# Fool-Yang/AlphaSnake-Zero

Hardware: AMD Instinct MI355X
Metric: self-play env-steps/sec (11x11, 4 snakes, 50 MCTS sims) (higher is better)
Workload: dtype f32 (tower convolutions: each f32 operand split into f16 hi + lo, 3 f16 MFMAs per product, f32 accumulate)

## Files before the change

### alphasnake-zero_amd/csrc/conv_split.hip

```cpp
#include "common.h"
#include "train_fold.h"
#include <stdlib.h>

typedef float f32x16 __attribute__((ext_vector_type(16)));
typedef _Float16 f16x8 __attribute__((ext_vector_type(8)));
typedef _Float16 f16x4 __attribute__((ext_vector_type(4)));
typedef __bf16 bf16x8 __attribute__((ext_vector_type(8)));
typedef unsigned uint4_t __attribute__((ext_vector_type(4)));
typedef int i32x4 __attribute__((ext_vector_type(4)));
typedef int i32x8 __attribute__((ext_vector_type(8)));
typedef short s16x2 __attribute__((ext_vector_type(2)));

template <bool BF> __device__ __forceinline__ float hs_from16(_Float16 v)
{
    if (BF) return (float)__builtin_bit_cast(__bf16, v);
    return (float)v;
}
template <bool BF> __device__ __forceinline__ _Float16 hs_to16(float v)
{
    if (BF) return __builtin_bit_cast(_Float16, (__bf16)v);
    return (_Float16)__builtin_amdgcn_fmed3f(v, -65504.f, 65504.f);
}

#define HS_C 128
// ... 1407 lines not shown
    SNK_REQUIRE(n_layers >= 1 && n_layers <= HS_RECT_MAX_LAYERS, "snk_conv_rect_plan: %d layers (at most %d)", n_layers, HS_RECT_MAX_LAYERS);
    const long mb = rect_max_blocks(n_images, height, width, act16);
    SNK_REQUIRE(mb >= 0 && mb < (1l << 31), "snk_conv_rect_plan: bad shape %d x %d x %d", n_images, height, width);
    if (n_images == 0) return 0;
    RectPlanArgs a;
    a.n_layers = n_layers;
    for (int i = 0; i < n_layers; ++i) {
        SNK_REQUIRE(grow[i] >= 0 && grow[i] < 128, "snk_conv_rect_plan: grow[%d] = %d", i, grow[i]);
        a.grow[i] = grow[i];
    }
    a.desc = (uint4 *)d_desc; a.max_blocks = mb; a.counts = d_counts;
    a.a16 = act16;
    hipStream_t st = (hipStream_t)stream;
    k_obs_bbox<<<(n_images + 3) / 4, 256, 0, st>>>(d_planes, n_images, height, width, b0, b1, b2, (unsigned *)d_bbox);
    k_rect_plan<<<n_layers, 1024, 0, st>>>((const unsigned *)d_bbox, n_images, height, width, a);
    SNK_CHECK_HIP(hipGetLastError());
    return 0;
}

extern "C" int snk_conv_rect_plan(const float *d_planes, float b0, float b1, float b2, int n_images, int height, int width,
                                  int n_layers, const int *grow, void *d_bbox, void *d_desc, int *d_counts, void *stream)
{
    return rect_plan(d_planes, b0, b1, b2, n_images, height, width, n_layers, grow, d_bbox, d_desc, d_counts, stream, false);
}

extern "C" int snk_conv_rect_plan_act16(const float *d_planes, float b0, float b1, float b2, int n_images, int height, int width,
                                        int n_layers, const int *grow, void *d_bbox, void *d_desc, int *d_counts, void *stream)
{
    return rect_plan(d_planes, b0, b1, b2, n_images, height, width, n_layers, grow, d_bbox, d_desc, d_counts, stream, true);
}


#define HS_PACK_BINS 4096
__host__ __device__ static inline bool hs_pack_fits(int wr, int Hd, int Wd, float inv, int m, int nA, int nB)
{
    const int yf = (int)(((float)m + 0.5f) * inv), yl = (int)(((float)(m + nA - 1) + 0.5f) * inv);
    const int cols_in = wr + 2 < Wd ? wr + 2 : Wd;
    int R = yl - yf + 3;
    int st = (R < Hd ? R : Hd) * cols_in;
    if (nB > 0) {
        const int RB = (int)(((float)(nB - 1) + 0.5f) * inv) + 3;
        R += RB;
        st += (RB < Hd ? RB : Hd) * cols_in;
    }
    return R * (wr + 2) <= HS_NPB_PK && st <= 64 * HS_NST;
}
__host__ __device__ static inline int hs_pack_period(int S) { const int t = S | 32, P = 32 / (t & -t); return P < 8 ? P : 8; }
template <class F> __host__ __device__ static inline void hs_pack_walk(int hr, int wr, int Hd, int Wd, int q, F &&emit)
{
    const int S = hr * wr;
    if (q == 1) {
        int tm;
        const int parts = hs_rect_parts(hr, wr, Hd, Wd, &tm), T = (S + 31) / 32, base = T / parts, rem = T % parts;
        for (int k = 0; k < parts; ++k) {
            const int tile0 = k * base + (k < rem ? k : rem), ntile = base + (k < rem ? 1 : 0);
            emit(0, 32 * tile0, 32 * (tile0 + ntile) < S ? 32 * ntile : S - 32 * tile0, 0, ntile);
        }
        return;
    }
    const float inv = 1.0f / (float)wr;
    int i = 0, m = 0;
    while (i < q) {
        const int left = (q - i) * S - m;
        const int rest = S - m;
        int nA = rest < 32 ? rest : 32, nB = 0;
        for (int n = 8; n >= 1; --n) {
            const int rows = 32 * n < left ? 32 * n : left;
            const int a_ = rows < rest ? rows : rest, b_ = rows - a_;
            if (b_ <= S && hs_pack_fits(wr, Hd, Wd, inv, m, a_, b_)) { nA = a_; nB = b_; break; }
        }
        emit(i, m, nA, nB, (nA + nB + 31) / 32);
        m += nA;
        if (m == S) { ++i; m = nB; if (m == S) { ++i; m = 0; } }
    }
}

__global__ __launch_bounds__(1024) void k_rect_plan_pack(const unsigned *__restrict__ bbox, int n, int Hd, int Wd, RectPlanArgs a,
                                                         int *__restrict__ order_all)
{
    __shared__ int cnt[HS_PACK_BINS], cur[HS_PACK_BINS], gb[HS_PACK_BINS + 1];
    __shared__ unsigned long long sc[1024];
    __shared__ int cls[9], clscur[9], tiles_sum;
    const int L = blockIdx.x, g = a.grow[L], tid = threadIdx.x, nb = Hd * Wd;
    int *order = order_all + (long)L * n;
    for (int b = tid; b < nb; b += 1024) cnt[b] = 0;
    if (tid < 9) cls[tid] = 0;
    if (tid == 0) tiles_sum = 0;
    __syncthreads();
#define HS_PACK_SHAPE(b_)                                                                       \
        const int y0 = max((int)((b_) & 255) - g, 0), x0 = max((int)(((b_) >> 8) & 255) - g, 0); \
        const int y1 = min((int)(((b_) >> 16) & 255) + g, Hd - 1), x1 = min((int)((b_) >> 24) + g, Wd - 1); \
        const int hr = y1 - y0 + 1, wr = x1 - x0 + 1, bin = (hr - 1) * Wd + wr - 1;
    for (int img = tid; img < n; img += 1024) {
        const unsigned b = bbox[img];
        HS_PACK_SHAPE(b)
        (void)y0; (void)x0;
        atomicAdd(&cnt[bin], 1);
    }
    __syncthreads();
    const int K = (nb + 1023) / 1024;
    unsigned long long mine = 0;
    for (int j = 0; j < K; ++j) {
        const int b = tid * K + j;
        if (b < nb && cnt[b] > 0) {
            const int P = hs_pack_period((b / Wd + 1) * (b % Wd + 1));
            mine += (unsigned long long)cnt[b] << 32 | (unsigned)((cnt[b] + P - 1) / P);
        }
    }
    sc[tid] = mine;
    __syncthreads();
    for (int s = 1; s < 1024; s <<= 1) {
        const unsigned long long v = tid >= s ? sc[tid - s] : 0ull;
        __syncthreads();
        sc[tid] += v;
        __syncthreads();
    }
    {
        unsigned long long e = sc[tid] - mine;
        for (int j = 0; j < K; ++j) {
            const int b = tid * K + j;
            if (b < nb) {
                cur[b] = (int)(e >> 32); gb[b] = (int)(e & 0xFFFFFFFFu);
                if (cnt[b] > 0) {
                    const int P = hs_pack_period((b / Wd + 1) * (b % Wd + 1));
                    e += (unsigned long long)cnt[b] << 32 | (unsigned)((cnt[b] + P - 1) / P);
                }
            }
        }
    }
    const int n_groups = (int)(sc[1023] & 0xFFFFFFFFu);
    if (tid == 0) gb[nb] = n_groups;
    __syncthreads();
    for (int img = tid; img < n; img += 1024) {
        const unsigned b = bbox[img];
        HS_PACK_SHAPE(b)
        (void)y0; (void)x0;
        order[atomicAdd(&cur[bin], 1)] = img;
    }
#undef HS_PACK_SHAPE
#define HS_PACK_GROUP(gi)                                                                       \
        int lo_ = 0, hi_ = nb;                                \
        while (lo_ < hi_) { const int mid_ = (lo_ + hi_) >> 1; if (gb[mid_ + 1] > (gi)) hi_ = mid_; else lo_ = mid_ + 1; } \
        const int bin = lo_, hr = bin / Wd + 1, wr = bin % Wd + 1, P = hs_pack_period(hr * wr);  \
        const int rank0 = ((gi) - gb[bin]) * P, q = min(P, cnt[bin] - rank0);
    int tiles = 0;
    for (int gi = tid; gi < n_groups; gi += 1024) {
        HS_PACK_GROUP(gi)
        hs_pack_walk(hr, wr, Hd, Wd, q, [&](int, int, int, int, int nt) { atomicAdd(&cls[nt], 1); tiles += nt; });
    }
    atomicAdd(&tiles_sum, tiles);
    __syncthreads();
    if (tid == 0) {
        int o = 0;
        for (int nt = 8; nt >= 1; --nt) { clscur[nt] = o; o += cls[nt]; }
        a.counts[2 * L] = 2 * o;
        a.counts[2 * L + 1] = tiles_sum;
    }
    __syncthreads();
    uint4 *desc = a.desc + (long)L * a.max_blocks;
    for (int gi = tid; gi < n_groups; gi += 1024) {
        HS_PACK_GROUP(gi)
        const int first = cur[bin] - cnt[bin] + rank0;
        hs_pack_walk(hr, wr, Hd, Wd, q, [&](int i, int m, int nA, int nB, int nt) {
            const int slot = atomicAdd(&clscur[nt], 1);
            desc[2 * slot] = make_uint4((unsigned)(first + i), 0u, (unsigned)m | (unsigned)nA << 16, 0u);
            desc[2 * slot + 1] = make_uint4((unsigned)(first + i + (nB > 0 ? 1 : 0)), 0u, (unsigned)nB | (unsigned)nt << 16, 0u);
        });
    }
#undef HS_PACK_GROUP
}

__global__ __launch_bounds__(256) void k_rect_pack_resolve(const unsigned *__restrict__ bbox, int n, int Hd, int Wd, RectPlanArgs a,
                                                           const int *__restrict__ order_all)
{
    const int L = blockIdx.y, e = blockIdx.x * 256 + threadIdx.x, g = a.grow[L];
    if (e >= a.counts[2 * L]) return;
    uint4 *d = a.desc + (long)L * a.max_blocks + e;
    const int img = order_all[(long)L * n + (int)d->x];
    const unsigned b = bbox[img];
    const int y0 = max((int)(b & 255) - g, 0), x0 = max((int)((b >> 8) & 255) - g, 0);
    const int y1 = min((int)((b >> 16) & 255) + g, Hd - 1), x1 = min((int)(b >> 24) + g, Wd - 1);
    d->x = (unsigned)img;
    d->y = (unsigned)y0 | (unsigned)x0 << 8 | (unsigned)(y1 - y0 + 1) << 16 | (unsigned)(x1 - x0 + 1) << 24;
    d->w = b;
}

static long rect_pack_max_desc(int n_images, int height, int width)
{
    if (n_images < 0 || height < 3 || width < 3 || height * width > HS_PACK_BINS) return -1;
    if (rect_max_parts(height, width, false) < 0) return -1;
    static int cache_h = 0, cache_w = 0;
    static double cache_r = 0.0;
    if (cache_h != height || cache_w != width) {
        double worst = 1.0;
        for (int hr = 1; hr <= height; ++hr)
            for (int wr = 1; wr <= width; ++wr) {
                const int P = hs_pack_period(hr * wr);
                int tm;
                const int alone = hs_rect_parts(hr, wr, height, width, &tm);
                if ((double)alone > worst) worst = (double)alone;
                if (P == 1) continue;
                int blocks = 0, done = 0;
                const int S = hr * wr;
                hs_pack_walk(hr, wr, height, width, P, [&](int i, int m, int nA, int nB, int) {
                    ++blocks;
                    const int upto = m + nA == S ? i + (nB == S ? 1 : 0) : -1;
                    for (; done <= upto && done < P; ++done) {
                        const double r = (double)blocks / (double)(done + 1);
                        if (r > worst) worst = r;
                    }
                });
            }
        cache_h = height; cache_w = width; cache_r = worst;
    }
    return 2 * ((long)((double)n_images * cache_r) + 1);
}

extern "C" long snk_conv_rect_pack_max_desc(int n_images, int height, int width) { return rect_pack_max_desc(n_images, height, width); }

extern "C" int snk_conv_rect_plan_pack(const float *d_planes, float b0, float b1, float b2, int n_images, int height, int width,
                                       int n_layers, const int *grow, void *d_bbox, void *d_desc, int *d_counts, void *d_order, void *stream)
{
    SNK_REQUIRE(d_planes && grow && d_bbox && d_desc && d_counts && d_order, "snk_conv_rect_plan_pack: NULL argument");
    SNK_REQUIRE(n_layers >= 1 && n_layers <= HS_RECT_MAX_LAYERS, "snk_conv_rect_plan_pack: %d layers (at most %d)", n_layers, HS_RECT_MAX_LAYERS);
    const long md = rect_pack_max_desc(n_images, height, width);
    SNK_REQUIRE(md >= 0 && md < (1l << 31), "snk_conv_rect_plan_pack: bad shape %d x %d x %d", n_images, height, width);
    if (n_images == 0) return 0;
    RectPlanArgs a;
    a.n_layers = n_layers;
    for (int i = 0; i < n_layers; ++i) {
        SNK_REQUIRE(grow[i] >= 0 && grow[i] < 128, "snk_conv_rect_plan_pack: grow[%d] = %d", i, grow[i]);
        a.grow[i] = grow[i];
    }
    a.desc = (uint4 *)d_desc; a.max_blocks = md; a.counts = d_counts;
    a.a16 = false;
    hipStream_t st = (hipStream_t)stream;
    k_obs_bbox<<<(n_images + 3) / 4, 256, 0, st>>>(d_planes, n_images, height, width, b0, b1, b2, (unsigned *)d_bbox);
    k_rect_plan_pack<<<n_layers, 1024, 0, st>>>((const unsigned *)d_bbox, n_images, height, width, a, (int *)d_order);
    k_rect_pack_resolve<<<dim3((unsigned)((md + 255) / 256), n_layers), 256, 0, st>>>((const unsigned *)d_bbox, n_images, height, width, a, (const int *)d_order);
    SNK_CHECK_HIP(hipGetLastError());
    return 0;
}

extern "C" int snk_conv_rect_plan_pack_host(const unsigned *h_bbox, int n_images, int height, int width, int grow,
                                            unsigned *h_desc, int *h_counts)
{
    SNK_REQUIRE(h_bbox && h_desc && h_counts, "snk_conv_rect_plan_pack_host: NULL argument");
    SNK_REQUIRE(grow >= 0 && grow < 128, "snk_conv_rect_plan_pack_host: grow = %d", grow);
    const long md = rect_pack_max_desc(n_images, height, width);
    SNK_REQUIRE(md >= 0 && md < (1l << 31), "snk_conv_rect_plan_pack_host: bad shape %d x %d x %d", n_images, height, width);
    const int nb = height * width;
    int *binof = (int *)malloc(sizeof(int) * (size_t)(n_images + 1)), *start = (int *)calloc((size_t)nb + 2, sizeof(int));
    int *order = (int *)malloc(sizeof(int) * (size_t)(n_images + 1));
    unsigned *rect = (unsigned *)malloc(sizeof(unsigned) * (size_t)(n_images + 1));
    unsigned *tmp = (unsigned *)malloc(16 * (size_t)(md + 2));
    long n_blk = 0, tiles = 0;
    bool ok = binof && start && order && rect && tmp;
    if (ok) {
        for (int i = 0; i < n_images; ++i) {
            const unsigned b = h_bbox[i];
            const int y0 = (int)(b & 255) - grow > 0 ? (int)(b & 255) - grow : 0, x0 = (int)((b >> 8) & 255) - grow > 0 ? (int)((b >> 8) & 255) - grow : 0;
            const int y1 = (int)((b >> 16) & 255) + grow < height - 1 ? (int)((b >> 16) & 255) + grow : height - 1;
            const int x1 = (int)(b >> 24) + grow < width - 1 ? (int)(b >> 24) + grow : width - 1;
            if (y1 < y0 || x1 < x0) { ok = false; break; }
            binof[i] = (y1 - y0) * width + x1 - x0;
            rect[i] = (unsigned)y0 | (unsigned)x0 << 8 | (unsigned)(y1 - y0 + 1) << 16 | (unsigned)(x1 - x0 + 1) << 24;
            ++start[binof[i] + 1];
        }
    }
    if (ok) {
        for (int b = 0; b < nb; ++b) start[b + 1] += start[b];
        for (int i = 0; i < n_images; ++i) order[start[binof[i]]++] = i;
// ... 334 lines not shown
```

### alphasnake-zero_amd/snake_engine/_lib.py

```python
import ctypes as C
import os

_HERE = os.path.dirname(os.path.abspath(__file__))
LIB_PATH = os.environ.get("SNK_LIB_PATH") or os.path.join(_HERE, "libsnake_engine.so")

MAX_SNAKES, MAX_CELLS, MAX_NODES = 8, 361, 384
ABI_VERSION = 113


class EngineError(RuntimeError):
    pass


class SnkGameState(C.Structure):
    _fields_ = [
        ("H", C.c_int32), ("W", C.c_int32), ("S", C.c_int32), ("uid", C.c_uint32),
        ("alive", C.c_uint8 * MAX_SNAKES),
        ("health", C.c_int16 * MAX_SNAKES),
        ("length", C.c_int16 * MAX_SNAKES),
        ("dir", C.c_uint8 * MAX_SNAKES),
        ("nodes", (C.c_int16 * MAX_NODES) * MAX_SNAKES),
        ("food", C.c_uint8 * MAX_CELLS),
        ("rewards", C.c_int8 * MAX_SNAKES),
        ("counters", C.c_int32 * 6),
# ... 22 lines not shown
    "snk_engine_observe": (i32, [vp, vp, i32, i32, vp, vp, vp, i32, vp]),
    "snk_engine_observe_rows": (i32, [vp, vp, vp, i32, i32, vp, vp, vp, i32, vp, vp, vp]),
    "snk_engine_export_sync": (i32, [vp, vp, i32, vp]),
    "snk_engine_import_sync": (i32, [vp, vp, i32, vp]),
    "snk_engine_import_at_sync": (i32, [vp, vp, i32, vp, i32]),
    "snk_engine_sum_counters_sync": (i32, [vp, vp, i32, vp]),
    "snk_compact_scratch_elems": (i32, [i32]),
    "snk_compact_flags": (i32, [vp, i32, vp, vp, vp, vp]),
    "snk_conv3x3_prepare_weights": (i32, [vp, vp, vp]),
    "snk_conv3x3_bn_f32": (i32, [vp, vp, vp, vp, vp, vp, i32, i32, i32, i32, vp]),
    "snk_conv3x3_prepare_weights_bf16": (i32, [vp, vp, vp]),
    "snk_conv3x3_prepare_weights_f16_act16": (i32, [vp, vp, vp]),
    "snk_conv3x3_bn_f16_act16_head": (i32, [vp, vp, vp, vp, vp, vp, C.c_float, C.c_float, vp, i32, i32, i32, vp]),
    "snk_conv3x3_bn_bf16_act16_head": (i32, [vp, vp, vp, vp, vp, vp, C.c_float, C.c_float, vp, i32, i32, i32, vp]),
    "snk_conv_rect_max_blocks_act16": (C.c_long, [i32, i32, i32]),
    "snk_conv_rect_plan_act16": (i32, [vp, C.c_float, C.c_float, C.c_float, i32, i32, i32, i32, C.POINTER(i32), vp, vp, vp, vp]),
    "snk_conv3x3_bn_bf16_act16": (i32, [vp, vp, vp, vp, vp, vp, i32, i32, i32, i32, i32, vp]),
    "snk_conv3x3_bn_bf16_act16_rect": (i32, [vp, vp, vp, vp, vp, vp, vp, vp, vp, i32, vp, i32, vp, i32, i32, i32, vp]),
    "snk_stem_conv_bn_relu_bf16out": (i32, [vp, vp, vp, vp, vp, i32, i32, i32, vp]),
    "snk_stem_conv_bn_relu_bf16out_rect": (i32, [vp, vp, vp, vp, vp, vp, i32, i32, i32, i32, vp]),
    "snk_conv3x3_prepare_weights_mxfp8": (i32, [vp, vp, vp]),
    "snk_conv3x3_bn_mxfp8_act16": (i32, [vp, vp, vp, vp, vp, vp, i32, i32, i32, i32, i32, vp]),
    "snk_conv3x3_bn_mxfp8_act16_rect": (i32, [vp, vp, vp, vp, vp, vp, vp, vp, vp, i32, vp, i32, vp, i32, i32, i32, vp]),
    "snk_conv3x3_bn_mxfp8_act16_head": (i32, [vp, vp, vp, vp, vp, vp, C.c_float, C.c_float, vp, i32, i32, i32, vp]),
    "snk_mxfp8_quantize_bf16": (i32, [vp, i32, vp, vp, vp]),
    "snk_conv3x3_prepare_weights_winograd": (i32, [vp, vp, vp]),
    "snk_conv3x3_bn_f32_winograd": (i32, [vp, vp, vp, vp, vp, vp, i32, i32, i32, i32, vp]),
    "snk_conv3x3_prepare_weights_f16s": (i32, [vp, vp, C.c_float, vp]),
    "snk_conv3x3_bn_f16s": (i32, [vp, vp, vp, vp, vp, vp, i32, i32, i32, i32, vp]),
    "snk_conv3x3_bn_f16": (i32, [vp, vp, vp, vp, vp, vp, i32, i32, i32, i32, vp]),
    "snk_conv_rect_max_blocks": (C.c_long, [i32, i32, i32]),
    "snk_conv_rect_plan": (i32, [vp, C.c_float, C.c_float, C.c_float, i32, i32, i32, i32, C.POINTER(i32), vp, vp, vp, vp]),
    "snk_conv_rect_pack_max_desc": (C.c_long, [i32, i32, i32]),
    "snk_conv_rect_plan_pack": (i32, [vp, C.c_float, C.c_float, C.c_float, i32, i32, i32, i32, C.POINTER(i32), vp, vp, vp, vp, vp]),
    "snk_conv_rect_plan_pack_host": (i32, [vp, i32, i32, i32, i32, vp, vp]),
    "snk_conv3x3_bn_f16s_rect_pack": (i32, [vp, vp, vp, vp, vp, vp, vp, vp, vp, i32, vp, i32, vp, i32, i32, i32, vp]),
    "snk_stem_conv_bn_relu_f32_rect": (i32, [vp, vp, vp, vp, vp, vp, i32, i32, i32, i32, vp]),
    "snk_stem_conv_bn_relu_f16out_rect": (i32, [vp, vp, vp, vp, vp, vp, i32, i32, i32, i32, vp]),
    "snk_conv3x3_bn_f16_act16_rect": (i32, [vp, vp, vp, vp, vp, vp, vp, vp, vp, i32, vp, i32, vp, i32, i32, i32, vp]),
    "snk_conv3x3_bn_f16s_rect": (i32, [vp, vp, vp, vp, vp, vp, vp, vp, vp, i32, vp, i32, vp, i32, i32, i32, vp]),
    "snk_conv3x3_bn_f16s_head": (i32, [vp, vp, vp, vp, vp, vp, vp, C.c_float, C.c_float, vp, i32, i32, i32, vp]),
    "snk_conv3x3_bn_f16_act16": (i32, [vp, vp, vp, vp, vp, vp, i32, i32, i32, i32, i32, vp]),
    "snk_stem_conv_bn_relu_f16out": (i32, [vp, vp, vp, vp, vp, i32, i32, i32, vp]),
    "snk_head_dense_f32": (i32, [vp, vp, vp, vp, vp, vp, vp, i32, i32, i32, vp]),
    "snk_stem_conv_bn_relu_f32": (i32, [vp, vp, vp, vp, vp, i32, i32, i32, vp]),
    "snk_tt_create": (i32, [C.POINTER(vp), u64, i32]),
    "snk_tt_destroy": (i32, [vp]),
    "snk_tt_clear": (i32, [vp, vp]),
    "snk_tt_status_sync": (i32, [vp, C.POINTER(C.c_int64), C.POINTER(C.c_int64), C.POINTER(i32)]),
    "snk_tt_rebuild_sync": (i32, [vp, u64, i32, i32]),
    "snk_tt_lookup_insert": (i32, [vp, vp, vp, i32, i32, i32, vp, vp, vp]),
    "snk_tt_find": (i32, [vp, vp, i32, i32, i32, vp, vp, vp]),
    "snk_tt_set_priors": (i32, [vp, vp, vp, i32, vp, vp, vp]),
    "snk_tt_read_q": (i32, [vp, vp, i32, i32, vp, vp]),
    "snk_mcts_select": (i32, [vp, vp, i32, C.c_float, vp, vp, C.c_int64, u64, C.c_uint32, C.c_uint32, vp, vp, vp, vp, vp, vp, i32, vp, vp]),
    "snk_mcts_gather_rows": (i32, [vp, i32, vp, vp, vp, vp, vp]),
    "snk_mcts_row_active": (i32, [vp, vp, i32, i32, vp, vp]),
    "snk_mcts_retire": (i32, [vp, vp, vp, i32, i32, vp, vp, vp]),
    "snk_mcts_backup": (i32, [vp, vp, i32, vp, vp, vp, vp, vp, i32, i32, vp, vp]),
    "snk_mcts_terminal_backup": (i32, [vp, vp, i32, vp, vp, vp, i32, i32, vp]),
    "snk_mcts_root_moves": (i32, [vp, vp, i32, C.c_float, i32, vp, vp, C.c_int64, u64, C.c_uint32, C.c_uint32, vp, vp]),
    "snk_softermax_argmax": (i32, [vp, i32, C.c_float, vp, vp, vp]),
    "snk_engine_rewards": (i32, [vp, vp, i32, vp, vp]),
    "snk_head_f32": (i32, [vp, vp, C.c_float, C.c_float, vp, vp, vp, vp, vp, vp, i32, i32, i32, vp]),
    "snk_bn_train_partials": (i32, []),
    "snk_conv3x3_f16s_input_scale": (i32, [vp, C.c_long, vp, vp, vp]),
    "snk_conv3x3_wgrad_partials": (C.c_long, [i32, i32]),
# ... 78 lines not shown
```

### alphasnake-zero_amd/snake_engine/net.py

```python
import ctypes as C
import math
import os

import numpy as np
import torch

from ._lib import lib, check, EngineError

BN_EPS = 1e-3
K_FILTERS = 128
F16S_WEIGHT_BYTES = 9 * 128 * 128 * 4 + 32
F16S_TAIL_OFFSET = 9 * 128 * 128 * 4
F16S_FLAG_OFFSET = F16S_TAIL_OFFSET + 16


def glorot_uniform_weights(input_shape, blocks=4, seed=0):
    g = torch.Generator().manual_seed(seed)
    h, w, c = input_shape
    k = K_FILTERS

    def glorot(shape, fan_in, fan_out):
        lim = math.sqrt(6.0 / (fan_in + fan_out))
        return ((torch.rand(shape, generator=g, dtype=torch.float32) * 2 - 1) * lim).numpy()

# ... 64 lines not shown
        g = i + 2
        ly = [min(h - 1, s + bh - 1 + g) - max(0, s - g) + 1 for s in range(h - bh + 1)]
        lx = [min(w - 1, s + bw - 1 + g) - max(0, s - g) + 1 for s in range(w - bw + 1)]
        if (sum(ly) / len(ly)) * (sum(lx) / len(lx)) >= threshold * h * w:
            break
        count += 1
    return count


class QNet:
    def __init__(self, weights, input_shape, device=None, max_chunk=4096):
        if not torch.cuda.is_available():
            raise EngineError("snake_engine.QNet needs an MI355X; there is no CPU fallback")
        self.L = lib()
        self.device = torch.device("cuda", torch.cuda.current_device() if device is None else int(device))
        self.input_shape = tuple(int(v) for v in input_shape)
        self.h, self.w, self.cin = self.input_shape
        assert self.cin == 3
        self.max_chunk = int(max_chunk)
        self._ws = None
        self.conv_timing = None
        self.clock_probe = None
        self.conv_algo = os.environ.get("SNK_CONV_ALGO", "f16s")
        if self.conv_algo not in ("f16s", "winograd", "direct", "bf16", "f16", "f16a", "mxfp8"):
            raise EngineError(f"SNK_CONV_ALGO={self.conv_algo!r}: expected f16s, winograd, direct, f16, f16a, bf16 or mxfp8")
        self.rect = self.conv_algo in ("f16s", "f16a", "bf16", "mxfp8") and os.environ.get("SNK_CONV_RECT", "1") != "0"
        self.act16 = {"f16a": torch.float16, "bf16": torch.bfloat16, "mxfp8": torch.bfloat16}.get(self.conv_algo)
        self.background = BACKGROUND_PIXEL
        self.guard_trips = 0
        self.rect_tiles = None
        self._bg = None
        self.rect_min = int(os.environ.get("SNK_CONV_RECT_MIN", "48"))
        self.rect_pack = os.environ.get("SNK_CONV_RECT_PACK", "1") != "0"
        self.n_streams = int(os.environ.get("SNK_NET_STREAMS", "1"))
        self._side = None
        self._guard = None
        self.set_weights(weights)

    def set_weights(self, weights):
        self.weights = [np.ascontiguousarray(w, np.float32) for w in weights]
        self.blocks = n_blocks_of(self.weights)
        dev = self.device
        t = [torch.as_tensor(w, device=dev) for w in self.weights]

        def fold(g, b, m, v):
            sc = g / torch.sqrt(v + BN_EPS)
            return sc.contiguous(), (b - m * sc).contiguous()
        self.stem_w = t[0].contiguous()
        self.stem_sc, self.stem_sh = fold(*t[1:5])
        self.conv_wT, self.conv_sc, self.conv_sh = [], [], []
        st = torch.cuda.current_stream().cuda_stream
        self.conv_x_scale = activation_scales(self.weights)
        self._wimg = None
        if self.conv_algo in ("f16s", "f16", "f16a", "bf16", "mxfp8") and self.blocks:
            self._wimg = torch.empty((2 * self.blocks, F16S_WEIGHT_BYTES), dtype=torch.uint8, device=dev)
            self._flags_host = torch.empty((2 * self.blocks,), dtype=torch.int32).pin_memory()
            if self._guard is None:
                self._guard = (torch.zeros((1,), dtype=torch.int32, device=dev), torch.zeros((1,), dtype=torch.int32).pin_memory())
        for i in range(2 * self.blocks):
            base = 5 + 5 * i
            if self.conv_algo == "bf16":
                self.conv_x_scale[i] = 1.0
                wT = self._wimg[i]
                check(self.L.snk_conv3x3_prepare_weights_bf16(t[base].contiguous().data_ptr(), wT.data_ptr(), st))
            elif self.conv_algo == "mxfp8":
                self.conv_x_scale[i] = 1.0
# ... 290 lines not shown
                       bufs[0].data_ptr(), m, self.h, self.w, st))
            bg = torch.empty((1 + self.n_rect, self.h, self.w, 128), dtype=dt, device=self.device)
            bg[0].copy_(bufs[0][0])
            cur, t1, t2 = bufs
            tm, self.conv_timing = self.conv_timing, None

            def conv(i, x, res, out):
                if a16:
                    check(self._fn16()[2](x.data_ptr(), self.conv_wT[i].data_ptr(), self.conv_sc[i].data_ptr(),
                                          self.conv_sh[i].data_ptr(), None if res is None else res.data_ptr(),
                                          out.data_ptr(), 1, m, self.h, self.w, 1, st))
                else:
                    self._conv(i, x, res, out, m, st)
            for i in range(self.n_rect):
                if i % 2 == 0:
                    conv(i, cur, None, t1)
                    bg[1 + i].copy_(t1[0])
                else:
                    conv(i, t1, cur, t2)
                    bg[1 + i].copy_(t2[0])
                    cur, t2 = t2, cur
            self.conv_timing = tm
            self._bg = bg
        return self._bg

    def _rect_args(self, i, plan, res):
        desc, counts, bg = plan[:3]
        return (desc[i].data_ptr(), counts[i].data_ptr(), bg[i].data_ptr(), i + 1,
                None if res is None else bg[i - 1].data_ptr(), i, bg[1 + i].data_ptr() if self.rect_fill[i] else None)

    def _use_rect(self, m):
        return self.n_rect > 0 and m >= self.rect_min

    def _rect_plan(self, x, m, k, st):
        bg = self.backgrounds()
        a16 = self.act16 is not None
        pack = not a16 and self.rect_pack and m * self.h * self.w * 128 < 2 ** 31
        mb = int(self.L.snk_conv_rect_pack_max_desc(m, self.h, self.w)) if pack else -1
        if mb < 0:
            pack = False
            mb = int((self.L.snk_conv_rect_max_blocks_act16 if a16 else self.L.snk_conv_rect_max_blocks)(m, self.h, self.w))
        if mb < 0:
            raise EngineError(f"sub-rectangle convolution: shape {m} x {self.h} x {self.w} not supported")
        key = ("rect", k)
        ws = None if self._ws is None else self._ws.get(key)
        if ws is None or ws[0].shape[0] != self.n_rect or ws[0].shape[1] < mb or ws[2].shape[0] < m:
            ws = (torch.empty((self.n_rect, mb, 4), dtype=torch.int32, device=self.device),
                  torch.zeros((self.n_rect, 2), dtype=torch.int32, device=self.device),
                  torch.empty((m,), dtype=torch.int32, device=self.device),
                  torch.empty((self.n_rect, m), dtype=torch.int32, device=self.device))
            if self._ws is None:
                self._ws = {}
            self._ws[key] = ws
        desc, counts, bbox, order = ws
        if self.rect_tiles is not None:
            counts = torch.zeros((self.n_rect, 2), dtype=torch.int32, device=self.device)
            self.rect_tiles.append((m, counts))
        grow = (C.c_int * self.n_rect)(*[i + 2 for i in range(self.n_rect)])
        desc_m = desc if desc.shape[1] == mb else desc.view(-1)[:self.n_rect * mb * 4].view(self.n_rect, mb, 4)
        b0, b1, b2 = self.background
        if pack:
            check(self.L.snk_conv_rect_plan_pack(x.data_ptr(), b0, b1, b2, m, self.h, self.w, self.n_rect, grow, bbox.data_ptr(),
                                                 desc_m.data_ptr(), counts.data_ptr(), order.data_ptr(), st))
            return desc_m, counts, bg, bbox, True
        check((self.L.snk_conv_rect_plan_act16 if a16 else self.L.snk_conv_rect_plan)(
            x.data_ptr(), b0, b1, b2, m, self.h, self.w, self.n_rect, grow, bbox.data_ptr(), desc_m.data_ptr(), counts.data_ptr(), st))
        return desc_m, counts, bg, bbox, False

    def _conv(self, i, x, res, out, m, st, h1=None, plan=None):
        tm = self.conv_timing
        if tm is not None:
            e0, e1 = torch.cuda.Event(enable_timing=True), torch.cuda.Event(enable_timing=True)
            e0.record(torch.cuda.current_stream())
        if plan is not None and i < self.n_rect and h1 is None:
            conv_rect = self.L.snk_conv3x3_bn_f16s_rect_pack if plan[4] else self.L.snk_conv3x3_bn_f16s_rect
            check(conv_rect(x.data_ptr(), self.conv_wT[i].data_ptr(), self.conv_sc[i].data_ptr(),
                            self.conv_sh[i].data_ptr(), None if res is None else res.data_ptr(),
                            out.data_ptr(), *self._rect_args(i, plan, res), m, self.h, self.w, st))
            if tm is not None:
                e1.record(torch.cuda.current_stream())
                tm.append((e0, e1, 2.0 * m * self.h * self.w * 9 * 128 * 128))
            return
        if h1 is not None:
            check(self.L.snk_conv3x3_bn_f16s_head(x.data_ptr(), self.conv_wT[i].data_ptr(), self.conv_sc[i].data_ptr(),
                                                  self.conv_sh[i].data_ptr(), None if res is None else res.data_ptr(),
                                                  None if out is None else out.data_ptr(), self.head_w.data_ptr(),
                                                  self.head_s, self.head_b, h1.data_ptr(), m, self.h, self.w, st))
            if tm is not None:
                e1.record(torch.cuda.current_stream())
                tm.append((e0, e1, 2.0 * m * self.h * self.w * 9 * 128 * 128))
            return
        fn = {"winograd": self.L.snk_conv3x3_bn_f32_winograd,
              "f16s": self.L.snk_conv3x3_bn_f16s, "f16": self.L.snk_conv3x3_bn_f16}.get(
            self.conv_algo, self.L.snk_conv3x3_bn_f32)
        check(fn(x.data_ptr(), self.conv_wT[i].data_ptr(), self.conv_sc[i].data_ptr(),
                 self.conv_sh[i].data_ptr(), None if res is None else res.data_ptr(),
# ... 29 lines not shown
```

### include/snake_engine.h

```cpp
#ifndef SNAKE_ENGINE_H
#define SNAKE_ENGINE_H

#include <stdint.h>

#ifdef __cplusplus
extern "C" {
#endif

#define SNK_MAX_SNAKES 8
#define SNK_MAX_CELLS 361
#define SNK_MAX_NODES 384

typedef struct snk_engine snk_engine;

typedef struct {
    int32_t H, W, S;
    uint32_t uid;
    uint8_t alive[SNK_MAX_SNAKES];
    int16_t health[SNK_MAX_SNAKES];
    int16_t length[SNK_MAX_SNAKES];
    uint8_t dir[SNK_MAX_SNAKES];
    int16_t nodes[SNK_MAX_SNAKES][SNK_MAX_NODES];
    uint8_t food[SNK_MAX_CELLS];
    int8_t rewards[SNK_MAX_SNAKES];
// ... 57 lines not shown
                                int height, int width, int relu, void *stream);
#define SNK_CONV_F16S_WEIGHT_BYTES (9 * 128 * 128 * 4 + 32)
#define SNK_CONV_F16S_TAIL_OFFSET (9 * 128 * 128 * 4)
#define SNK_CONV_F16S_FLAG_OFFSET (9 * 128 * 128 * 4 + 16)
int snk_conv3x3_prepare_weights_f16s(const float *d_w_hwio, void *d_wS, float x_scale, void *stream);
int snk_conv3x3_f16s_set_guard_word(void *d_wS, int32_t *d_word, void *stream);
int snk_conv3x3_bn_f16s(const float *d_x, const void *d_wS, const float *d_scale, const float *d_shift,
                        const float *d_residual, float *d_out, int n_images, int height, int width, int relu,
                        void *stream);
int snk_conv3x3_bn_f16(const float *d_x, const void *d_wS, const float *d_scale, const float *d_shift,
                       const float *d_residual, float *d_out, int n_images, int height, int width, int relu,
                       void *stream);
long snk_conv_rect_max_blocks(int n_images, int height, int width);
int snk_conv_rect_plan(const float *d_planes, float b0, float b1, float b2, int n_images, int height, int width,
                       int n_layers, const int *grow, void *d_bbox, void *d_desc, int *d_counts, void *stream);
int snk_stem_conv_bn_relu_f32_rect(const float *d_x, const float *d_w, const float *d_scale, const float *d_shift,
                                   float *d_out, const void *d_bbox, int grow, int n_images, int height, int width,
                                   void *stream);
long snk_conv_rect_max_blocks_act16(int n_images, int height, int width);
int snk_conv_rect_plan_act16(const float *d_planes, float b0, float b1, float b2, int n_images, int height, int width,
                             int n_layers, const int *grow, void *d_bbox, void *d_desc, int *d_counts, void *stream);
int snk_stem_conv_bn_relu_f16out_rect(const float *d_x, const float *d_w, const float *d_scale, const float *d_shift,
                                      void *d_out16, const void *d_bbox, int grow, int n_images, int height, int width,
                                      void *stream);
int snk_conv3x3_bn_f16_act16_rect(const void *d_x16, const void *d_wS, const float *d_scale, const float *d_shift,
                                  const void *d_residual16, void *d_out16, const void *d_desc, const int *d_count,
                                  const void *d_bg_in16, int grow_in, const void *d_bg_res16, int grow_res,
                                  const void *d_bg_out16, int n_images, int height, int width, void *stream);
int snk_conv3x3_bn_f16s_rect(const float *d_x, const void *d_wS, const float *d_scale, const float *d_shift,
                             const float *d_residual, float *d_out, const void *d_desc, const int *d_count,
                             const float *d_bg_in, int grow_in, const float *d_bg_res, int grow_res,
                             const float *d_bg_out, int n_images, int height, int width, void *stream);
long snk_conv_rect_pack_max_desc(int n_images, int height, int width);
int snk_conv_rect_plan_pack(const float *d_planes, float b0, float b1, float b2, int n_images, int height, int width,
                            int n_layers, const int *grow, void *d_bbox, void *d_desc, int *d_counts, void *d_order, void *stream);
int snk_conv_rect_plan_pack_host(const unsigned *h_bbox, int n_images, int height, int width, int grow,
                                 unsigned *h_desc, int *h_counts);
int snk_conv3x3_bn_f16s_rect_pack(const float *d_x, const void *d_wS, const float *d_scale, const float *d_shift,
                                  const float *d_residual, float *d_out, const void *d_desc, const int *d_count,
                                  const float *d_bg_in, int grow_in, const float *d_bg_res, int grow_res,
                                  const float *d_bg_out, int n_images, int height, int width, void *stream);
int snk_conv3x3_bn_f16s_head(const float *d_x, const void *d_wS, const float *d_scale, const float *d_shift,
                             const float *d_residual, float *d_out, const float *d_w1x1, float bn_scale,
                             float bn_shift, float *d_h1, int n_images, int height, int width, void *stream);
int snk_conv3x3_prepare_weights_f16_act16(const float *d_w_hwio, void *d_wS, void *stream);
int snk_conv3x3_bn_f16_act16(const void *d_x16, const void *d_wS, const float *d_scale, const float *d_shift,
                             const void *d_residual16, void *d_out, int out_f16, int n_images, int height, int width,
                             int relu, void *stream);
int snk_stem_conv_bn_relu_f16out(const float *d_x, const float *d_w, const float *d_scale, const float *d_shift,
                                 void *d_out16, int n_images, int height, int width, void *stream);
int snk_conv3x3_prepare_weights_bf16(const float *d_w_hwio, void *d_wS, void *stream);
int snk_conv3x3_bn_bf16_act16(const void *d_x16, const void *d_wS, const float *d_scale, const float *d_shift,
                              const void *d_residual16, void *d_out, int out_bf16, int n_images, int height, int width,
                              int relu, void *stream);
int snk_conv3x3_bn_bf16_act16_rect(const void *d_x16, const void *d_wS, const float *d_scale, const float *d_shift,
                                   const void *d_residual16, void *d_out16, const void *d_desc, const int *d_count,
                                   const void *d_bg_in16, int grow_in, const void *d_bg_res16, int grow_res,
                                   const void *d_bg_out16, int n_images, int height, int width, void *stream);
int snk_conv3x3_bn_f16_act16_head(const void *d_x16, const void *d_wS, const float *d_scale, const float *d_shift,
                                  const void *d_residual16, const float *d_w1x1, float bn_scale, float bn_shift,
                                  float *d_h1, int n_images, int height, int width, void *stream);
int snk_conv3x3_bn_bf16_act16_head(const void *d_x16, const void *d_wS, const float *d_scale, const float *d_shift,
                                   const void *d_residual16, const float *d_w1x1, float bn_scale, float bn_shift,
                                   float *d_h1, int n_images, int height, int width, void *stream);
int snk_stem_conv_bn_relu_bf16out(const float *d_x, const float *d_w, const float *d_scale, const float *d_shift,
                                  void *d_out16, int n_images, int height, int width, void *stream);
int snk_stem_conv_bn_relu_bf16out_rect(const float *d_x, const float *d_w, const float *d_scale, const float *d_shift,
                                       void *d_out16, const void *d_bbox, int grow, int n_images, int height, int width,
// ... 165 lines not shown
```

Measured before the change: 1037.

## Precompute packed-rect cut templates on host and parallelize plan emission

Replaces the per-call walk of each packing group inside a single 1024-thread block with a precomputed table of cuts per (bin, group size), built once on the host and uploaded. The bin kernel now reads block and tile counts from the table and sorts image order with a shared-memory bitonic sort. A new grid-wide emit kernel computes descriptors directly, and the separate resolve pass is removed. This targets the serial planning cost on the critical path of each inference batch, at the cost of a larger order buffer and a device-resident table.

New measurement: 1037 (median of 4 runs). Within noise of the previous version (-0.0%).

```diff
diff --git a/alphasnake-zero_amd/csrc/conv_split.hip b/alphasnake-zero_amd/csrc/conv_split.hip
--- a/alphasnake-zero_amd/csrc/conv_split.hip
+++ b/alphasnake-zero_amd/csrc/conv_split.hip
@@ -1463,6 +1463,7 @@
 
 
 #define HS_PACK_BINS 4096
+#define HS_PACK_SORT 8192
 __host__ __device__ static inline bool hs_pack_fits(int wr, int Hd, int Wd, float inv, int m, int nA, int nB)
 {
     const int yf = (int)(((float)m + 0.5f) * inv), yl = (int)(((float)(m + nA - 1) + 0.5f) * inv);
@@ -1506,14 +1507,111 @@
     }
 }
 
-__global__ __launch_bounds__(1024) void k_rect_plan_pack(const unsigned *__restrict__ bbox, int n, int Hd, int Wd, RectPlanArgs a,
-                                                         int *__restrict__ order_all)
-{
-    __shared__ int cnt[HS_PACK_BINS], cur[HS_PACK_BINS], gb[HS_PACK_BINS + 1];
+#define HS_TPL_HEAD 4
+__host__ __device__ static inline uint4 hs_tpl_head(const unsigned *t, int bin, int q)
+{
+    const unsigned *h = t + HS_TPL_HEAD + 4 * (8 * bin + q - 1);
+    return make_uint4(h[0], h[1], h[2], h[3]);
+}
+__host__ __device__ static inline uint2 hs_tpl_block(const unsigned *t, int nb, const uint4 head, int j)
+{
+    const unsigned *b = t + HS_TPL_HEAD + 32 * nb + 2 * (head.x + (unsigned)j);
+    return make_uint2(b[0], b[1]);
+}
+__host__ __device__ static inline int hs_tpl_class(const uint4 head, int nt) { return (int)(((nt <= 4 ? head.z : head.w) >> (8 * ((nt - 1) & 3))) & 255u); }
+__host__ __device__ static inline int hs_tpl_bin_blocks(const unsigned *t, int bin, int P, int cnt)
+{
+    const int r = cnt % P;
+    return (cnt / P) * (int)(hs_tpl_head(t, bin, P).y & 0xFFFFu) + (r ? (int)(hs_tpl_head(t, bin, r).y & 0xFFFFu) : 0);
+}
+__host__ __device__ static inline uint2 hs_tpl_bin_block(const unsigned *t, int nb, int bin, int P, int cnt, int k, int *rank0)
+{
+    const uint4 hP = hs_tpl_head(t, bin, P);
+    const int nP = (int)(hP.y & 0xFFFFu), G = cnt / P;
+    const int g = k / nP < G ? k / nP : G;
+    *rank0 = g * P;
+    return hs_tpl_block(t, nb, g < G ? hP : hs_tpl_head(t, bin, cnt - G * P), k - g * nP);
+}
+
+static long rect_pack_templates(int height, int width, unsigned *h_tab, long cap)
+{
+    if (height < 3 || width < 3 || height * width > HS_PACK_BINS) return -1;
+    if (rect_max_parts(height, width, false) < 0) return -1;
+    const int nb = height * width;
+    const long base = HS_TPL_HEAD + 32l * nb;
+    long nblk = 0;
+    bool ok = true;
+    if (h_tab) {
+        if (cap < base) return -1;
+        for (long k = 0; k < base; ++k) h_tab[k] = 0u;
+    }
+    for (int bin = 0; bin < nb; ++bin) {
+        const int hr = bin / width + 1, wr = bin % width + 1;
+        for (int q = 1; q <= 8; ++q) {
+            unsigned cls[9] = {0, 0, 0, 0, 0, 0, 0, 0, 0}, tiles = 0, n = 0;
+            const long first = nblk;
+            hs_pack_walk(hr, wr, height, width, q, [&](int i, int m, int nA, int nB, int nt) {
+                if (m > 0xFFFF || nA > 0xFFFF || nB > 0xFFFF || nt < 1 || nt > 8 || i > 7) ok = false;
+                if (h_tab && base + 2 * (nblk + 1) <= cap) {
+                    h_tab[base + 2 * nblk] = (unsigned)m | (unsigned)nA << 16;
+                    h_tab[base + 2 * nblk + 1] = (unsigned)nB | (unsigned)nt << 16 | (unsigned)i << 24;
+                }
+                if (nt >= 1 && nt <= 8) ++cls[nt];
+                tiles += (unsigned)nt; ++n; ++nblk;
+            });
+            for (int nt = 1; nt <= 8; ++nt) if (cls[nt] > 255u) ok = false;
+            if (n > 0xFFFFu || tiles > 0xFFFFu) ok = false;
+            if (h_tab) {
+                unsigned *h = h_tab + HS_TPL_HEAD + 4 * (8 * bin + q - 1);
+                h[0] = (unsigned)first; h[1] = n | tiles << 16;
+                h[2] = cls[1] | cls[2] << 8 | cls[3] << 16 | cls[4] << 24; h[3] = cls[5] | cls[6] << 8 | cls[7] << 16 | cls[8] << 24;
+            }
+        }
+    }
+    const long words = base + 2 * nblk;
+    if (!ok || words >= (1l << 31)) return -1;
+    if (h_tab) {
+        if (cap < words) return -1;
+        h_tab[0] = (unsigned)height; h_tab[1] = (unsigned)width; h_tab[2] = (unsigned)words; h_tab[3] = (unsigned)nblk;
+    }
+    return words;
+}
+
+extern "C" long snk_conv_rect_pack_templates(int height, int width, unsigned *h_tab, long cap_words)
+{
+    return rect_pack_templates(height, width, h_tab, cap_words);
+}
+
+extern "C" int snk_conv_rect_pack_template_cut(const unsigned *h_tab, int hr, int wr, int q, int *h_out, int cap_blocks)
+{
+    SNK_REQUIRE(h_tab && h_out, "snk_conv_rect_pack_template_cut: NULL argument");
+    const int Hd = (int)h_tab[0], Wd = (int)h_tab[1];
+    SNK_REQUIRE(hr >= 1 && hr <= Hd && wr >= 1 && wr <= Wd && q >= 1 && q <= 8,
+                "snk_conv_rect_pack_template_cut: no group of %d images of %d x %d on a %d x %d canvas", q, hr, wr, Hd, Wd);
+    const int bin = (hr - 1) * Wd + wr - 1, n = hs_tpl_bin_blocks(h_tab, bin, q, q);
+    SNK_REQUIRE(n <= cap_blocks, "snk_conv_rect_pack_template_cut: %d blocks, room for %d", n, cap_blocks);
+    for (int k = 0; k < n; ++k) {
+        int rank0;
+        const uint2 b = hs_tpl_bin_block(h_tab, Hd * Wd, bin, q, q, k, &rank0);
+        h_out[5 * k] = rank0 + (int)(b.y >> 24); h_out[5 * k + 1] = (int)(b.x & 0xFFFFu); h_out[5 * k + 2] = (int)(b.x >> 16);
+        h_out[5 * k + 3] = (int)(b.y & 0xFFFFu); h_out[5 * k + 4] = (int)((b.y >> 16) & 15u);
+    }
+    return n;
+}
+
+__host__ __device__ static inline long hs_pack_order_ints(int n, int nb) { return (long)n + 2 * nb + 1 + 16; }
+
+__global__ __launch_bounds__(1024) void k_rect_pack_bins(const unsigned *__restrict__ bbox, int n, int Hd, int Wd, RectPlanArgs a,
+                                                         int *__restrict__ order_all, const unsigned *__restrict__ tpl)
+{
+    __shared__ int cnt[HS_PACK_BINS];
+    __shared__ unsigned keys[HS_PACK_SORT];
     __shared__ unsigned long long sc[1024];
-    __shared__ int cls[9], clscur[9], tiles_sum;
+    __shared__ int cls[9], tiles_sum;
+    static_assert(HS_PACK_SORT >= HS_PACK_BINS && HS_PACK_SORT <= (1 << 13) && HS_PACK_BINS <= (1 << 12), "a key is bin << 13 | image");
+    int *cur = (int *)keys;
     const int L = blockIdx.x, g = a.grow[L], tid = threadIdx.x, nb = Hd * Wd;
-    int *order = order_all + (long)L * n;
+    int *order = order_all + (long)L * hs_pack_order_ints(n, nb), *binblk = order + n, *binfirst = binblk + nb + 1, *clscur = binfirst + nb;
     for (int b = tid; b < nb; b += 1024) cnt[b] = 0;
     if (tid < 9) cls[tid] = 0;
     if (tid == 0) tiles_sum = 0;
@@ -1521,23 +1619,30 @@
 #define HS_PACK_SHAPE(b_)                                                                       \
         const int y0 = max((int)((b_) & 255) - g, 0), x0 = max((int)(((b_) >> 8) & 255) - g, 0); \
         const int y1 = min((int)(((b_) >> 16) & 255) + g, Hd - 1), x1 = min((int)((b_) >> 24) + g, Wd - 1); \
-        const int hr = y1 - y0 + 1, wr = x1 - x0 + 1, bin = (hr - 1) * Wd + wr - 1;
+        const int bin = (y1 - y0) * Wd + x1 - x0;
     for (int img = tid; img < n; img += 1024) {
         const unsigned b = bbox[img];
         HS_PACK_SHAPE(b)
-        (void)y0; (void)x0;
         atomicAdd(&cnt[bin], 1);
     }
     __syncthreads();
     const int K = (nb + 1023) / 1024;
     unsigned long long mine = 0;
+    int tiles = 0;
     for (int j = 0; j < K; ++j) {
         const int b = tid * K + j;
         if (b < nb && cnt[b] > 0) {
-            const int P = hs_pack_period((b / Wd + 1) * (b % Wd + 1));
-            mine += (unsigned long long)cnt[b] << 32 | (unsigned)((cnt[b] + P - 1) / P);
-        }
-    }
+            const int P = hs_pack_period((b / Wd + 1) * (b % Wd + 1)), G = cnt[b] / P, r = cnt[b] - G * P;
+            const uint4 hP = hs_tpl_head(tpl, b, P), hr_ = r ? hs_tpl_head(tpl, b, r) : make_uint4(0u, 0u, 0u, 0u);
+            mine += (unsigned long long)cnt[b] << 32 | (unsigned)(G * (int)(hP.y & 0xFFFFu) + (int)(hr_.y & 0xFFFFu));
+            tiles += G * (int)(hP.y >> 16) + (int)(hr_.y >> 16);
+            for (int nt = 1; nt <= 8; ++nt) {
+                const int c = G * hs_tpl_class(hP, nt) + hs_tpl_class(hr_, nt);
+                if (c) atomicAdd(&cls[nt], c);
+            }
+        }
+    }
+    if (tiles) atomicAdd(&tiles_sum, tiles);
     sc[tid] = mine;
     __syncthreads();
     for (int s = 1; s < 1024; s <<= 1) {
@@ -1551,69 +1656,91 @@
         for (int j = 0; j < K; ++j) {
             const int b = tid * K + j;
             if (b < nb) {
-                cur[b] = (int)(e >> 32); gb[b] = (int)(e & 0xFFFFFFFFu);
-                if (cnt[b] > 0) {
-                    const int P = hs_pack_period((b / Wd + 1) * (b % Wd + 1));
-                    e += (unsigned long long)cnt[b] << 32 | (unsigned)((cnt[b] + P - 1) / P);
-                }
+                cur[b] = (int)(e >> 32); binfirst[b] = (int)(e >> 32); binblk[b] = (int)(e & 0xFFFFFFFFu);
+                if (cnt[b] > 0) e += (unsigned long long)cnt[b] << 32 | (unsigned)hs_tpl_bin_blocks(tpl, b, hs_pack_period((b / Wd + 1) * (b % Wd + 1)), cnt[b]);
             }
         }
     }
-    const int n_groups = (int)(sc[1023] & 0xFFFFFFFFu);
-    if (tid == 0) gb[nb] = n_groups;
-    __syncthreads();
-    for (int img = tid; img < n; img += 1024) {
-        const unsigned b = bbox[img];
-        HS_PACK_SHAPE(b)
-        (void)y0; (void)x0;
-        order[atomicAdd(&cur[bin], 1)] = img;
-    }
-#undef HS_PACK_SHAPE
-#define HS_PACK_GROUP(gi)                                                                       \
-        int lo_ = 0, hi_ = nb;                                \
-        while (lo_ < hi_) { const int mid_ = (lo_ + hi_) >> 1; if (gb[mid_ + 1] > (gi)) hi_ = mid_; else lo_ = mid_ + 1; } \
-        const int bin = lo_, hr = bin / Wd + 1, wr = bin % Wd + 1, P = hs_pack_period(hr * wr);  \
-        const int rank0 = ((gi) - gb[bin]) * P, q = min(P, cnt[bin] - rank0);
-    int tiles = 0;
-    for (int gi = tid; gi < n_groups; gi += 1024) {
-        HS_PACK_GROUP(gi)
-        hs_pack_walk(hr, wr, Hd, Wd, q, [&](int, int, int, int, int nt) { atomicAdd(&cls[nt], 1); tiles += nt; });
-    }
-    atomicAdd(&tiles_sum, tiles);
-    __syncthreads();
     if (tid == 0) {
+        const int n_blocks = (int)(sc[1023] & 0xFFFFFFFFu);
+        binblk[nb] = n_blocks;
         int o = 0;
         for (int nt = 8; nt >= 1; --nt) { clscur[nt] = o; o += cls[nt]; }
-        a.counts[2 * L] = 2 * o;
+        a.counts[2 * L] = 2 * n_blocks;
         a.counts[2 * L + 1] = tiles_sum;
     }
     __syncthreads();
-    uint4 *desc = a.desc + (long)L * a.max_blocks;
-    for (int gi = tid; gi < n_groups; gi += 1024) {
-        HS_PACK_GROUP(gi)
-        const int first = cur[bin] - cnt[bin] + rank0;
-        hs_pack_walk(hr, wr, Hd, Wd, q, [&](int i, int m, int nA, int nB, int nt) {
-            const int slot = atomicAdd(&clscur[nt], 1);
-            desc[2 * slot] = make_uint4((unsigned)(first + i), 0u, (unsigned)m | (unsigned)nA << 16, 0u);
-            desc[2 * slot + 1] = make_uint4((unsigned)(first + i + (nB > 0 ? 1 : 0)), 0u, (unsigned)nB | (unsigned)nt << 16, 0u);
-        });
-    }
-#undef HS_PACK_GROUP
-}
-
-__global__ __launch_bounds__(256) void k_rect_pack_resolve(const unsigned *__restrict__ bbox, int n, int Hd, int Wd, RectPlanArgs a,
-                                                           const int *__restrict__ order_all)
-{
-    const int L = blockIdx.y, e = blockIdx.x * 256 + threadIdx.x, g = a.grow[L];
-    if (e >= a.counts[2 * L]) return;
-    uint4 *d = a.desc + (long)L * a.max_blocks + e;
-    const int img = order_all[(long)L * n + (int)d->x];
-    const unsigned b = bbox[img];
-    const int y0 = max((int)(b & 255) - g, 0), x0 = max((int)((b >> 8) & 255) - g, 0);
-    const int y1 = min((int)((b >> 16) & 255) + g, Hd - 1), x1 = min((int)(b >> 24) + g, Wd - 1);
-    d->x = (unsigned)img;
-    d->y = (unsigned)y0 | (unsigned)x0 << 8 | (unsigned)(y1 - y0 + 1) << 16 | (unsigned)(x1 - x0 + 1) << 24;
-    d->w = b;
+    if (n <= HS_PACK_SORT) {
+        int N = 64;
+        while (N < n) N <<= 1;
+        for (int i = tid; i < N; i += 1024) {
+            unsigned key = 0xFFFFFFFFu;
+            if (i < n) { const unsigned b = bbox[i]; HS_PACK_SHAPE(b) key = (unsigned)bin << 13 | (unsigned)i; }
+            keys[i] = key;
+        }
+        __syncthreads();
+        for (int k = 2; k <= N; k <<= 1)
+            for (int j = k >> 1; j > 0; j >>= 1) {
+                for (int p = tid; p < (N >> 1); p += 1024) {
+                    const int i = ((p & ~(j - 1)) << 1) | (p & (j - 1)), l = i | j;
+                    const unsigned x = keys[i], y = keys[l];
+                    if ((x > y) == ((i & k) == 0)) { keys[i] = y; keys[l] = x; }
+                }
+                __syncthreads();
+            }
+        for (int i = tid; i < n; i += 1024) order[i] = (int)(keys[i] & (unsigned)(HS_PACK_SORT - 1));
+    } else {
+        for (int img = tid; img < n; img += 1024) {
+            const unsigned b = bbox[img];
+            HS_PACK_SHAPE(b)
+            order[atomicAdd(&cur[bin], 1)] = img;
+        }
+    }
+#undef HS_PACK_SHAPE
+}
+
+__global__ __launch_bounds__(256) void k_rect_pack_emit(const unsigned *__restrict__ bbox, int n, int Hd, int Wd, RectPlanArgs a,
+                                                        int *__restrict__ order_all, const unsigned *__restrict__ tpl)
+{
+    __shared__ int sb[HS_PACK_BINS + 1];
+    __shared__ int cls[9], clsbase[9];
+    const int L = blockIdx.y, g = a.grow[L], tid = threadIdx.x, nb = Hd * Wd, e = blockIdx.x * 256 + tid;
+    int *order = order_all + (long)L * hs_pack_order_ints(n, nb), *binblk = order + n, *binfirst = binblk + nb + 1, *clscur = binfirst + nb;
+    const int n_blocks = a.counts[2 * L] >> 1;
+    if ((int)blockIdx.x * 256 >= n_blocks) return;
+    for (int b = tid; b <= nb; b += 256) sb[b] = binblk[b];
+    if (tid < 9) cls[tid] = 0;
+    __syncthreads();
+    uint4 dA = make_uint4(0u, 0u, 0u, 0u), dB = dA;
+    int nt = 0, rank = 0;
+    if (e < n_blocks) {
+        int lo = 0, hi = nb;
+        while (lo < hi) { const int mid = (lo + hi) >> 1; if (sb[mid + 1] > e) hi = mid; else lo = mid + 1; }
+        const int bin = lo, P = hs_pack_period((bin / Wd + 1) * (bin % Wd + 1)), first = binfirst[bin];
+        const int cntb = (bin + 1 < nb ? binfirst[bin + 1] : n) - first;
+        int rank0;
+        const uint2 t = hs_tpl_bin_block(tpl, nb, bin, P, cntb, e - sb[bin], &rank0);
+        const int pa = first + rank0 + (int)(t.y >> 24), nB = (int)(t.y & 0xFFFFu);
+        const int ia = order[pa], ib = nB > 0 ? order[pa + 1] : ia;
+        const unsigned ba = bbox[ia], bb = bbox[ib];
+        nt = (int)((t.y >> 16) & 15u);
+#define HS_PACK_RECT(b_)                                                                        \
+        ((unsigned)max((int)((b_) & 255) - g, 0) | (unsigned)max((int)(((b_) >> 8) & 255) - g, 0) << 8 | \
+         (unsigned)(min((int)(((b_) >> 16) & 255) + g, Hd - 1) - max((int)((b_) & 255) - g, 0) + 1) << 16 | \
+         (unsigned)(min((int)((b_) >> 24) + g, Wd - 1) - max((int)(((b_) >> 8) & 255) - g, 0) + 1) << 24)
+        dA = make_uint4((unsigned)ia, HS_PACK_RECT(ba), t.x, ba);
+        dB = make_uint4((unsigned)ib, HS_PACK_RECT(bb), t.y & 0xFFFFFFu, bb);
+#undef HS_PACK_RECT
+        rank = atomicAdd(&cls[nt], 1);
+    }
+    __syncthreads();
+    if (tid >= 1 && tid <= 8) clsbase[tid] = cls[tid] ? atomicAdd(&clscur[tid], cls[tid]) : 0;
+    __syncthreads();
+    if (e < n_blocks) {
+        uint4 *desc = a.desc + (long)L * a.max_blocks + 2l * (clsbase[nt] + rank);
+        desc[0] = dA;
+        desc[1] = dB;
+    }
 }
 
 static long rect_pack_max_desc(int n_images, int height, int width)
@@ -1649,26 +1776,34 @@
 
 extern "C" long snk_conv_rect_pack_max_desc(int n_images, int height, int width) { return rect_pack_max_desc(n_images, height, width); }
 
-extern "C" int snk_conv_rect_plan_pack(const float *d_planes, float b0, float b1, float b2, int n_images, int height, int width,
-                                       int n_layers, const int *grow, void *d_bbox, void *d_desc, int *d_counts, void *d_order, void *stream)
-{
-    SNK_REQUIRE(d_planes && grow && d_bbox && d_desc && d_counts && d_order, "snk_conv_rect_plan_pack: NULL argument");
-    SNK_REQUIRE(n_layers >= 1 && n_layers <= HS_RECT_MAX_LAYERS, "snk_conv_rect_plan_pack: %d layers (at most %d)", n_layers, HS_RECT_MAX_LAYERS);
+extern "C" long snk_conv_rect_pack_order_ints(int n_images, int height, int width)
+{
+    if (rect_pack_max_desc(n_images, height, width) < 0) return -1;
+    return hs_pack_order_ints(n_images, height * width);
+}
+
+extern "C" int snk_conv_rect_plan_pack_tab(const float *d_planes, float b0, float b1, float b2, int n_images, int height, int width,
+                                       int n_layers, const int *grow, void *d_bbox, void *d_desc, int *d_counts, void *d_order,
+                                       const void *d_templ, void *stream)
+{
+    SNK_REQUIRE(d_planes && grow && d_bbox && d_desc && d_counts && d_order && d_templ, "snk_conv_rect_plan_pack_tab: NULL argument");
+    SNK_REQUIRE(n_layers >= 1 && n_layers <= HS_RECT_MAX_LAYERS, "snk_conv_rect_plan_pack_tab: %d layers (at most %d)", n_layers, HS_RECT_MAX_LAYERS);
     const long md = rect_pack_max_desc(n_images, height, width);
-    SNK_REQUIRE(md >= 0 && md < (1l << 31), "snk_conv_rect_plan_pack: bad shape %d x %d x %d", n_images, height, width);
+    SNK_REQUIRE(md >= 0 && md < (1l << 31), "snk_conv_rect_plan_pack_tab: bad shape %d x %d x %d", n_images, height, width);
     if (n_images == 0) return 0;
     RectPlanArgs a;
     a.n_layers = n_layers;
     for (int i = 0; i < n_layers; ++i) {
-        SNK_REQUIRE(grow[i] >= 0 && grow[i] < 128, "snk_conv_rect_plan_pack: grow[%d] = %d", i, grow[i]);
+        SNK_REQUIRE(grow[i] >= 0 && grow[i] < 128, "snk_conv_rect_plan_pack_tab: grow[%d] = %d", i, grow[i]);
         a.grow[i] = grow[i];
     }
     a.desc = (uint4 *)d_desc; a.max_blocks = md; a.counts = d_counts;
     a.a16 = false;
     hipStream_t st = (hipStream_t)stream;
     k_obs_bbox<<<(n_images + 3) / 4, 256, 0, st>>>(d_planes, n_images, height, width, b0, b1, b2, (unsigned *)d_bbox);
-    k_rect_plan_pack<<<n_layers, 1024, 0, st>>>((const unsigned *)d_bbox, n_images, height, width, a, (int *)d_order);
-    k_rect_pack_resolve<<<dim3((unsigned)((md + 255) / 256), n_layers), 256, 0, st>>>((const unsigned *)d_bbox, n_images, height, width, a, (const int *)d_order);
+    k_rect_pack_bins<<<n_layers, 1024, 0, st>>>((const unsigned *)d_bbox, n_images, height, width, a, (int *)d_order, (const unsigned *)d_templ);
+    k_rect_pack_emit<<<dim3((unsigned)((md / 2 + 255) / 256), n_layers), 256, 0, st>>>((const unsigned *)d_bbox, n_images, height, width, a, (int *)d_order,
+                                                                                      (const unsigned *)d_templ);
     SNK_CHECK_HIP(hipGetLastError());
     return 0;
 }
diff --git a/alphasnake-zero_amd/snake_engine/_lib.py b/alphasnake-zero_amd/snake_engine/_lib.py
--- a/alphasnake-zero_amd/snake_engine/_lib.py
+++ b/alphasnake-zero_amd/snake_engine/_lib.py
@@ -78,7 +78,10 @@
     "snk_conv_rect_max_blocks": (C.c_long, [i32, i32, i32]),
     "snk_conv_rect_plan": (i32, [vp, C.c_float, C.c_float, C.c_float, i32, i32, i32, i32, C.POINTER(i32), vp, vp, vp, vp]),
     "snk_conv_rect_pack_max_desc": (C.c_long, [i32, i32, i32]),
-    "snk_conv_rect_plan_pack": (i32, [vp, C.c_float, C.c_float, C.c_float, i32, i32, i32, i32, C.POINTER(i32), vp, vp, vp, vp, vp]),
+    "snk_conv_rect_pack_order_ints": (C.c_long, [i32, i32, i32]),
+    "snk_conv_rect_pack_templates": (C.c_long, [i32, i32, vp, C.c_long]),
+    "snk_conv_rect_pack_template_cut": (i32, [vp, i32, i32, i32, vp, i32]),
+    "snk_conv_rect_plan_pack_tab": (i32, [vp, C.c_float, C.c_float, C.c_float, i32, i32, i32, i32, C.POINTER(i32), vp, vp, vp, vp, vp, vp]),
     "snk_conv_rect_plan_pack_host": (i32, [vp, i32, i32, i32, i32, vp, vp]),
     "snk_conv3x3_bn_f16s_rect_pack": (i32, [vp, vp, vp, vp, vp, vp, vp, vp, vp, i32, vp, i32, vp, i32, i32, i32, vp]),
     "snk_stem_conv_bn_relu_f32_rect": (i32, [vp, vp, vp, vp, vp, vp, i32, i32, i32, i32, vp]),
diff --git a/alphasnake-zero_amd/snake_engine/net.py b/alphasnake-zero_amd/snake_engine/net.py
--- a/alphasnake-zero_amd/snake_engine/net.py
+++ b/alphasnake-zero_amd/snake_engine/net.py
@@ -120,6 +120,7 @@
         self._bg = None
         self.rect_min = int(os.environ.get("SNK_CONV_RECT_MIN", "48"))
         self.rect_pack = os.environ.get("SNK_CONV_RECT_PACK", "1") != "0"
+        self._pack_tab = None
         self.n_streams = int(os.environ.get("SNK_NET_STREAMS", "1"))
         self._side = None
         self._guard = None
@@ -476,6 +477,17 @@
     def _use_rect(self, m):
         return self.n_rect > 0 and m >= self.rect_min
 
+    def _pack_templates(self):
+        if self._pack_tab is None:
+            words = int(self.L.snk_conv_rect_pack_templates(self.h, self.w, None, 0))
+            if words < 0:
+                raise EngineError(f"packed sub-rectangle plan: canvas {self.h} x {self.w} not supported")
+            tab = np.zeros((words,), dtype=np.uint32)
+            if int(self.L.snk_conv_rect_pack_templates(self.h, self.w, tab.ctypes.data_as(C.c_void_p), words)) != words:
+                raise EngineError("packed sub-rectangle plan: the table of cuts could not be built")
+            self._pack_tab = torch.from_numpy(tab.view(np.int32)).to(self.device)
+        return self._pack_tab
+
     def _rect_plan(self, x, m, k, st):
         bg = self.backgrounds()
         a16 = self.act16 is not None
@@ -489,10 +501,11 @@
         key = ("rect", k)
         ws = None if self._ws is None else self._ws.get(key)
         if ws is None or ws[0].shape[0] != self.n_rect or ws[0].shape[1] < mb or ws[2].shape[0] < m:
+            oi = max(int(self.L.snk_conv_rect_pack_order_ints(m, self.h, self.w)), 1)
             ws = (torch.empty((self.n_rect, mb, 4), dtype=torch.int32, device=self.device),
                   torch.zeros((self.n_rect, 2), dtype=torch.int32, device=self.device),
                   torch.empty((m,), dtype=torch.int32, device=self.device),
-                  torch.empty((self.n_rect, m), dtype=torch.int32, device=self.device))
+                  torch.empty((self.n_rect * oi,), dtype=torch.int32, device=self.device))
             if self._ws is None:
                 self._ws = {}
             self._ws[key] = ws
@@ -504,8 +517,9 @@
         desc_m = desc if desc.shape[1] == mb else desc.view(-1)[:self.n_rect * mb * 4].view(self.n_rect, mb, 4)
         b0, b1, b2 = self.background
         if pack:
-            check(self.L.snk_conv_rect_plan_pack(x.data_ptr(), b0, b1, b2, m, self.h, self.w, self.n_rect, grow, bbox.data_ptr(),
-                                                 desc_m.data_ptr(), counts.data_ptr(), order.data_ptr(), st))
+            check(self.L.snk_conv_rect_plan_pack_tab(x.data_ptr(), b0, b1, b2, m, self.h, self.w, self.n_rect, grow, bbox.data_ptr(),
+                                                 desc_m.data_ptr(), counts.data_ptr(), order.data_ptr(),
+                                                 self._pack_templates().data_ptr(), st))
             return desc_m, counts, bg, bbox, True
         check((self.L.snk_conv_rect_plan_act16 if a16 else self.L.snk_conv_rect_plan)(
             x.data_ptr(), b0, b1, b2, m, self.h, self.w, self.n_rect, grow, bbox.data_ptr(), desc_m.data_ptr(), counts.data_ptr(), st))
diff --git a/include/snake_engine.h b/include/snake_engine.h
--- a/include/snake_engine.h
+++ b/include/snake_engine.h
@@ -113,8 +113,12 @@
                              const float *d_bg_in, int grow_in, const float *d_bg_res, int grow_res,
                              const float *d_bg_out, int n_images, int height, int width, void *stream);
 long snk_conv_rect_pack_max_desc(int n_images, int height, int width);
-int snk_conv_rect_plan_pack(const float *d_planes, float b0, float b1, float b2, int n_images, int height, int width,
-                            int n_layers, const int *grow, void *d_bbox, void *d_desc, int *d_counts, void *d_order, void *stream);
+long snk_conv_rect_pack_order_ints(int n_images, int height, int width);
+long snk_conv_rect_pack_templates(int height, int width, unsigned *h_tab, long cap_words);
+int snk_conv_rect_pack_template_cut(const unsigned *h_tab, int hr, int wr, int q, int *h_out, int cap_blocks);
+int snk_conv_rect_plan_pack_tab(const float *d_planes, float b0, float b1, float b2, int n_images, int height, int width,
+                            int n_layers, const int *grow, void *d_bbox, void *d_desc, int *d_counts, void *d_order,
+                            const void *d_templ, void *stream);
 int snk_conv_rect_plan_pack_host(const unsigned *h_bbox, int n_images, int height, int width, int grow,
                                  unsigned *h_desc, int *h_counts);
 int snk_conv3x3_bn_f16s_rect_pack(const float *d_x, const void *d_wS, const float *d_scale, const float *d_shift,
```
